# lightonai/next-plaid

Hardware: AMD Instinct MI355X
Metric: queries/sec + p50 latency, k=10, 10M-doc x 300-tok x d128 PLAID index, 1/2/4/8 GPU (higher is better)
Workload: dtype f32 (split-bf16 hi/lo MFMA on the residual term of MaxSim, f32-class accuracy)

## Files before the change

### next-plaid_amd/csrc/np_index.hip

```cpp
#include "np_internal.h"

#include <hipcub/hipcub.hpp>

#include <algorithm>
#include <memory>
#include <thread>
#include <math.h>
#include <stdio.h>
#include <time.h>
#include <stdlib.h>
#include <string.h>

namespace np {

int DevBuf::reserve(size_t bytes) {
  if (bytes <= cap) return NP_OK;
  if (p) (void)hipFree(p);
  p = nullptr;
  cap = 0;
  size_t want = bytes + (bytes >> 3) + 256;
  hipError_t e = hipMalloc(&p, want);
  if (e != hipSuccess) {
    p = nullptr;
    set_error("hipMalloc(%zu bytes) failed: %s", want, hipGetErrorString(e));
    return NP_ERR_OUT_OF_MEMORY;
  }
  cap = want;
  return NP_OK;
}
void DevBuf::release() {
  if (p) (void)hipFree(p);
  p = nullptr;
  cap = 0;
}

void shard_range(int64_t n_total, int rank, int count, int64_t* b, int64_t* e) {
  if (count <= 1) {
    *b = 0;
    *e = n_total;
    return;
  }
  *b = (int64_t)((__int128)n_total * rank / count);
  *e = (int64_t)((__int128)n_total * (rank + 1) / count);
}

int normalise_opts(const np_open_opts* in, np_open_opts* o) {
  memset(o, 0, sizeof *o);
  if (in) *o = *in;
  if (o->shard_count <= 0) o->shard_count = 1;
  if (o->shard_rank < 0 || o->shard_rank >= o->shard_count) {
    set_error("Invalid configuration: shard_rank %d out of range for shard_count %d", o->shard_rank, o->shard_count);
    return NP_ERR_INVALID_ARGUMENT;
  }
  if (o->n_contexts <= 0) o->n_contexts = 2;
  if (o->n_contexts > 16) o->n_contexts = 16;
  if (o->max_batch <= 0) o->max_batch = 64;
  if (o->max_query_tokens <= 0) o->max_query_tokens = 64;
  return NP_OK;
}

bool set_tuning(Tuning* t, const std::string& n, int value) {
  auto clamp = [](int v, int lo, int hi) { return std::min(std::max(v, lo), hi); };
  if (n == "s4_mode") t->s4_mode = clamp(value, 0, 8);
  else if (n == "s4_minb") t->s4_minb = std::max(value, 1);
  else if (n == "s4_nbx") t->s4_nbx = clamp(value, 8, 512);
  else if (n == "s4_swz") t->s4_swz = value != 0;
  else if (n == "s4_filter") t->s4_filter = value != 0;
  else if (n == "s4_hot") t->s4_hot = clamp(value, 0, 500);
  else if (n == "s4_planes") t->s4_planes = value != 0;
  else if (n == "s4_pexp") t->s4_pexp = clamp(value, 5, 40);
  else if (n == "s4_lpd") t->s4_lpd = value == 2 ? 2 : 4;
  else if (n == "s4_qm") t->s4_qm = value != 0;
  else if (n == "s4_pnbx") t->s4_pnbx = clamp(value, 8, 512);
  else if (n == "s3_slices") t->s3_slices = value != 0;
  else if (n == "s4_warm") t->s4_warm = clamp(value, 0, 1000);
  else if (n == "ub_ncut") t->ub_ncut = clamp(value, 1, 512);
  else if (n == "s3_bisect") t->s3_bisect = clamp(value, 0, 1);
  else if (n == "s3_gain") t->s3_gain = clamp(value, 0, 2);
  else if (n == "s3_gain_mult") t->s3_gain_mult = clamp(value, 1, 16);
  else if (n == "s3_gain_direct") t->s3_gain_direct = clamp(value, 0, 64);
  else if (n == "s4_hot_auto") t->s4_hot_auto = clamp(value, 0, 0x7fffffff);
  else if (n == "ub_nt") t->ub_nt = value < 0 || value > 2 ? 0 : value;
  else if (n == "ub_steal") t->ub_steal = value < 1 ? 1 : value;
  else if (n == "ub_nbx") t->ub_nbx = clamp(value, 8, 256);
  else if (n == "ub_direct") t->ub_direct = clamp(value, 0, 16);
#ifdef NP_DIAGNOSTICS
  else if (n == "s4_probe") t->s4_probe = clamp(value, 0, 7);
#endif
  else if (n == "ub_static") t->ub_static = value != 0;
  else if (n == "hot_static") t->hot_static = value != 0;
  else if (n == "s6_xcd") t->s6_xcd = value != 0;
  else if (n == "s6_tiles") t->s6_tiles = value != 0;
  else if (n == "s6_lds") t->s6_lds = clamp(value, 0, 2);
  else if (n == "gemm_cpw") t->gemm_cpw = value == 2 ? 2 : 1;
  else if (n == "s1_split") t->s1_split = value != 0;
  else if (n == "exact_rowmax") t->exact_rowmax = value != 0;
  else return false;
  return true;
}

void read_tuning_env(Tuning* t) {
  static const char* const knobs[][2] = {
      {"NP_S4_MODE", "s4_mode"}, {"NP_S4_MINB", "s4_minb"}, {"NP_S4_NBX", "s4_nbx"}, {"NP_S4_SWZ", "s4_swz"},
      {"NP_S4_FILTER", "s4_filter"}, {"NP_S4_HOT", "s4_hot"}, {"NP_S4_PLANES", "s4_planes"}, {"NP_S4_PEXP", "s4_pexp"}, {"NP_S4_LPD", "s4_lpd"}, {"NP_S4_QM", "s4_qm"}, {"NP_S4_PNBX", "s4_pnbx"}, {"NP_S4_WARM", "s4_warm"}, {"NP_UB_NCUT", "ub_ncut"}, {"NP_S3_BISECT", "s3_bisect"}, {"NP_S3_GAIN", "s3_gain"}, {"NP_S3_GAIN_MULT", "s3_gain_mult"}, {"NP_S3_GAIN_DIRECT", "s3_gain_direct"}, {"NP_S4_HOT_AUTO", "s4_hot_auto"}, {"NP_S3_SLICES", "s3_slices"}, {"NP_UB_NT", "ub_nt"},
      {"NP_UB_STEAL", "ub_steal"}, {"NP_UB_NBX", "ub_nbx"}, {"NP_UB_DIRECT", "ub_direct"}, {"NP_UB_STATIC", "ub_static"}, {"NP_HOT_STATIC", "hot_static"}, {"NP_S6_XCD", "s6_xcd"}, {"NP_S6_TILES", "s6_tiles"}, {"NP_S6_LDS", "s6_lds"}, {"NP_GEMM_CPW", "gemm_cpw"}, {"NP_S1_SPLIT", "s1_split"},
      {"NP_EXACT_ROWMAX", "exact_rowmax"}};
  for (const auto& k : knobs) {
    const char* e = getenv(k[0]);
    if (e && *e) (void)set_tuning(t, k[1], atoi(e));
  }
#ifdef NP_DIAGNOSTICS
  if (const char* e = getenv("NP_S4_PROBE")) (void)set_tuning(t, "s4_probe", atoi(e));
#endif
}

static void default_workspace(DeviceIndex* ix) {
  ix->ws_auto = ix->opts.workspace_bytes <= 0;
  ix->ws_budget = ix->opts.workspace_bytes;
  ix->ws_budget_open = ix->opts.workspace_bytes;
  if (!ix->ws_auto) return;
  size_t free_b = 0, total_b = 0;
  int64_t ws = (int64_t)8 << 30;
  if (hipMemGetInfo(&free_b, &total_b) == hipSuccess) {
    const int64_t share = ((int64_t)free_b - ((int64_t)4 << 30)) / std::max(ix->opts.n_contexts, 1);
    ws = std::min<int64_t>((int64_t)16 << 30, std::max<int64_t>((int64_t)2 << 30, share));
  }
  ix->opts.workspace_bytes = ws;
  ix->ws_budget = ws;
  ix->ws_budget_open = ws;
}

static int check_device(int dev) {
  int n = 0;
  if (hipGetDeviceCount(&n) != hipSuccess || n <= 0) {
    (void)hipGetLastError();
    set_error("no HIP device available");
    return NP_ERR_DEVICE_UNAVAILABLE;
  }
  if (dev < 0 || dev >= n) {
    set_error("device %d out of range (%d devices)", dev, n);
    return NP_ERR_DEVICE_UNAVAILABLE;
  }
  return NP_OK;
}

void destroy_device_index(np_index* ix) {
  if (!ix) return;
  DeviceGuard g(ix->device);
  for (Context* c : ix->contexts) destroy_context(c);
  delete ix;
}

struct CloseIndex {
  void operator()(np_index* p) const { destroy_device_index(p); }
};
using IndexHandle = std::unique_ptr<np_index, CloseIndex>;

static uint32_t bitrev(uint32_t v, int nbits) {
  uint32_t r = 0;
  for (int k = 0; k < nbits; ++k)
    if (v & (1u << k)) r |= 1u << (nbits - 1 - k);
  return r;
}

static int check_geometry(int64_t K, int dim, int nbits, int64_t n_total) {
  if (nbits <= 0 || 8 % nbits != 0) {
    set_error("Codec error: nbits must be a divisor of 8, got %d", nbits);
    return NP_ERR_CODEC;
  }
  if (K <= 0 || dim <= 0) {
    set_error("Shape error: centroids must be [K > 0, dim > 0], got [%lld, %d]", (long long)K, dim);
    return NP_ERR_SHAPE;
  }
  if ((dim * nbits) % 8 != 0) {
    set_error("Shape error: dim*nbits must be a multiple of 8 (dim=%d nbits=%d)", dim, nbits);
    return NP_ERR_SHAPE;
  }
  if (K >= ((int64_t)1 << 31) || n_total >= ((int64_t)1 << 32) - 1) {
    set_error("Index load failed: K=%lld / N=%lld exceed the 32-bit device id space", (long long)K, (long long)n_total);
    return NP_ERR_INDEX_LOAD;
  }
  return NP_OK;
}

__global__ void __launch_bounds__(256) centroid_bound_kernel(const float* __restrict__ C, int64_t K, int dim,
                                                             uint32_t* __restrict__ out ) {
  const int64_t c = (int64_t)blockIdx.x * 4 + (threadIdx.x >> 6);
// ... 1450 lines not shown
```

### next-plaid_amd/csrc/np_internal.h

```cpp
#pragma once
#include <hip/hip_runtime.h>
#include <stdint.h>
#include <algorithm>
#include <atomic>
#include <mutex>
#include <condition_variable>
#include <string>
#include <vector>
#include "../../include/nextplaid_hip.h"

namespace np {

struct CodeArr {
  const void* p;
  int wide;
  __device__ __forceinline__ uint32_t operator[](int64_t i) const {
    return wide ? static_cast<const uint32_t*>(p)[i] : (uint32_t)static_cast<const uint16_t*>(p)[i];
  }
};

void set_error(const char* fmt, ...) __attribute__((format(printf, 1, 2)));
const char* last_error();
void clear_error();

// ... 60 lines not shown
int build_check_finite(const float* x, int64_t count, int dim);
int find_outliers(int device, const float* X, int64_t n, int dim, const float* C, int64_t k, float thr,
                  std::vector<int64_t>* out, int64_t* n_rechecked);
int kmeans_points_as_docs(int device, const float* pts, int64_t n, int dim, const np_index_config& cfg, int64_t k,
                          std::vector<float>* cen);
int encode_with_codec(int device, const float* C, int64_t K, int dim, int nbits, const float* weights, const float* cutoffs,
                      const float* X, int64_t T, int64_t* codes, uint8_t* packed, float* norms);
float quantile_of_sorted(const std::vector<float>& v, double q);

template <class T>
class DevPtr {
 public:
  DevPtr() = default;
  DevPtr(DevPtr&& o) noexcept : p_(o.p_) { o.p_ = nullptr; }
  DevPtr& operator=(DevPtr&& o) noexcept {
    if (this != &o) {
      reset();
      p_ = o.p_;
      o.p_ = nullptr;
    }
    return *this;
  }
  ~DevPtr() { reset(); }
  int alloc(size_t n, size_t* acct = nullptr) {
    reset();
    const size_t bytes = std::max<size_t>(n, 1) * sizeof(T);
    hipError_t e = hipMalloc((void**)&p_, bytes);
    if (e != hipSuccess) {
      p_ = nullptr;
      set_error("hipMalloc(%zu bytes) failed: %s", bytes, hipGetErrorString(e));
      return NP_ERR_OUT_OF_MEMORY;
    }
    if (acct) *acct += bytes;
    return NP_OK;
  }
  T* get() const { return p_; }
  void reset() {
    if (p_) (void)hipFree(p_);
    p_ = nullptr;
  }

 private:
  T* p_ = nullptr;
};

struct DevBuf {
  void* p = nullptr;
  size_t cap = 0;
  int reserve(size_t bytes);
  void release();
  template <class T> T* as() const { return (T*)p; }
};

struct Workspace;

struct Context {
  hipStream_t stream = nullptr;
  hipEvent_t ev[10] = {};
  Workspace* ws = nullptr;
  bool busy = false;
  uint64_t last_use = 0;
};

struct Tuning {
  int s4_mode = 4;
  int s4_minb = 8;
  int s4_nbx = 128;
  int s4_swz = 1;
  int s3_bisect = 1;
  int s3_slices = 1;
  int s3_gain = 1;
  int s3_gain_mult = 3;
  int s3_gain_direct = 16;
  int s4_filter = 1;
  int s4_hot = 60;
  int s4_hot_auto = 200000;
  int s4_planes = 1;
  int s4_lpd = 2;
  int s4_pnbx = 96;
  int s4_qm = 1;
  int s4_pexp = 15;
  int s4_warm = 0;
  int ub_ncut = 96;
  int ub_direct = 8;
  int hot_static = 1;
  int ub_static = 0;
  int s4_probe = 0;
  int ub_nbx = 96;
  int ub_steal = 16384;
  int ub_nt = 2;
  int s6_xcd = 1;
  int s6_lds = 1;
  int s6_tiles = 1;
  int s1_split = 0;
  int gemm_cpw = 1;
  int exact_rowmax = 0;
};

#define NP_IVF_SPLIT_RANGE 32768

struct DeviceIndex {
  int device = 0;
  int64_t N_total = 0, n_emb_total = 0;
  double avg_doclen = 0.0;
  int64_t doc_begin = 0, n_docs = 0;
  int64_t K = 0, KP = 0;
  int32_t dim = 0, nbits = 0, pd = 0;
  int32_t ldim = 0, lnbits = 0, lpd = 0;
  float pad_ss = 0.f;
  int64_t T = 0;
  int64_t max_doc_len = 0;
  DevPtr<float> d_centroids;
  DevPtr<float> d_wlut;
  DevPtr<uint8_t> d_codes;
  int code_wide = 0;
  DevPtr<uint8_t> d_ucodes;
  int64_t n_ucodes = 0;
  int ublock_stride = 0;
  int ublock_hdr = 0;
  DevPtr<int32_t> d_ulen;
  DevPtr<uint4> d_useg;
  DevPtr<uint4> d_doc_meta;
  float ulen_mean = 0.f;
  bool sliced_ok = false;
  float cmax = 0.f;
  bool filter_ok = false;
  bool s6_fast_ok = false;
  DevPtr<float> d_inv_norm;
  DevPtr<uint16_t> d_tok_pos;
  bool tok_sorted = false;
  DevPtr<uint8_t> d_residuals;
  DevPtr<int64_t> d_doc_offsets;
  DevPtr<uint32_t> d_ivf;
  DevPtr<int64_t> d_ivf_offsets;
  int64_t ivf_size = 0;
  bool ivf_sorted = false;
  DevPtr<uint32_t> d_ivf_split;
  int n_ranges = 0;
  std::vector<int64_t> ivf_top_prefix;
  size_t device_bytes = 0;
  np_open_opts opts{};
  mutable std::atomic<int64_t> ws_budget{0};
  int64_t ws_budget_open = 0;
  bool ws_auto = false;
  Tuning tune;
  mutable std::atomic<int> gain_skip{0};
  mutable std::atomic<int> gain_run{0};
  mutable std::atomic<uint64_t> gain_key{0};
  CodeArr codes() const { return CodeArr{d_codes.get(), code_wide}; }
  CodeArr ucodes() const { return CodeArr{d_ucodes.get(), code_wide}; }
  size_t code_bytes() const { return code_wide ? 4 : 2; }
  mutable std::mutex mu;
  mutable std::condition_variable cv;
  mutable std::vector<Context*> contexts;
  mutable uint64_t use_clock = 0;
};

static inline int storage_dim(int dim) { return dim <= 0 || dim > 128 ? dim : (dim + 31) / 32 * 32; }
static inline int storage_nbits(int dim, int nbits) { return (nbits == 1 && dim <= 128) ? 2 : nbits; }

int build_device_index(const HostIndex& h, const np_open_opts* opts, DeviceIndex** out);
void destroy_device_index(np_index* ix);
int normalise_opts(const np_open_opts* in, np_open_opts* out);
void read_tuning_env(Tuning* t);
bool set_tuning(Tuning* t, const std::string& name, int value);
void shard_range(int64_t n_total, int rank, int count, int64_t* b, int64_t* e);
// ... 28 lines not shown
```

### next-plaid_amd/csrc/np_kernels.h

```cpp
#pragma once
#include <hip/hip_runtime.h>
#include <stdint.h>

namespace np {

typedef float f32x16 __attribute__((ext_vector_type(16)));
typedef __bf16 bf16x8 __attribute__((ext_vector_type(8)));

#define NP_NEG_INF (-__builtin_huge_valf())
#define NP_MAX_QT 8

__device__ __forceinline__ uint32_t okey(float x) {
  uint32_t b = __float_as_uint(x);
  uint32_t k = (b & 0x80000000u) ? ~b : (b | 0x80000000u);
  return ((b & 0x7F800000u) == 0x7F800000u) ? 0u : k;
}
__device__ __forceinline__ float unkey(uint32_t k) {
  uint32_t b = (k & 0x80000000u) ? (k ^ 0x80000000u) : ~k;
  return __uint_as_float(b);
}
__device__ __forceinline__ bool finitef(float x) { return (__float_as_uint(x) & 0x7F800000u) != 0x7F800000u; }
__device__ __forceinline__ float readlane_f(float v, int lane) {
  return __int_as_float(__builtin_amdgcn_readlane(__float_as_int(v), lane));
}
// ... 2418 lines not shown
          }
        };
        uint4 va[8], vb[8];
        issue(0, va);
        int t = 0;
        for (; t + 16 < np; t += 16) {
          issue(t + 8, vb);
          fold(va);
          issue(t + 16, va);
          fold(vb);
        }
        if (t + 8 < np) {
          issue(t + 8, vb);
          fold(va);
          fold(vb);
        } else {
          fold(va);
        }
      }
      uint32_t sum = 0;
      int slo = 0;
      if constexpr (FLOOR) {
        uint32_t fl = lam2;
        int lq_here = Lq - 16 * jl;
        asm volatile("" : "+v"(fl), "+v"(lq_here));
#pragma unroll
        for (int k = 0; k < 16; ++k) {
          slo += (int)st[k] - ((k < lq_here && st[k] <= 1u) ? 254 : 0);
          sum += max(st[k], k < lq_here ? fl : 0u);
        }
      } else {
#pragma unroll
        for (int k = 0; k < 16; ++k) {
          sum += st[k];
          slo += (int)st[k] - (st[k] == 1u ? 254 : 0);
        }
      }
#pragma unroll
      for (int o = 1; o < LPD; o <<= 1) {
        sum += (uint32_t)__shfl_xor((int)sum, o);
        slo += __shfl_xor(slo, o);
      }
      const uint32_t sum_lo = (uint32_t)max(slo, 0);
      if (valid && jl == 0) {
        U[pbase + i] = (uint16_t)sum;
        if (hb) atomicAdd(&s_hist[min(sum_lo >> hshift, (uint32_t)(NP_UB_BINS - 1))], 1u);
      }
      __builtin_amdgcn_wave_barrier();
    }
    __syncthreads();
    if (hb)
      for (int i = tid; i < NP_UB_BINS; i += 256) {
        const uint32_t v = s_hist[i];
        if (v) atomicAdd(&hb[i], v);
      }
  }
#pragma unroll
  for (int o = 32; o > 0; o >>= 1) {
    toks += __shfl_xor(toks, o);
    ucnt += __shfl_xor(ucnt, o);
    ndoc += __shfl_xor(ndoc, o);
  }
  __shared__ unsigned long long s_cnt[3];
  __syncthreads();
  if (tid == 0) s_cnt[0] = s_cnt[1] = s_cnt[2] = 0;
  __syncthreads();
  if (lane == 0 && toks) {
    atomicAdd(&s_cnt[0], toks);
    atomicAdd(&s_cnt[1], ucnt);
    atomicAdd(&s_cnt[2], ndoc);
  }
  __syncthreads();
  if (tid == 0 && s_cnt[0] && ctr) {
    if (count_tokens) {
      atomicAdd(&ctr->n_cand_tokens, s_cnt[0]);
      atomicAdd(&ctr->n_cand_dcodes, s_cnt[1]);
    } else {
      atomicAdd(&ctr->n_level2, s_cnt[2]);
    }
    atomicAdd(&ctr->n_cand_codes, s_cnt[1]);
  }
}

__global__ void __launch_bounds__(256) ub_thr_kernel(const uint32_t* __restrict__ hist, int hshift, int slack, int n_sel,
                                                     const int32_t* __restrict__ n_cand, RoundPlan rp, int round,
                                                     const uint32_t* __restrict__ qflag, uint32_t* __restrict__ thr) {
  __shared__ uint32_t s_part[256];
  constexpr int BPT = NP_UB_BINS / 256;
  const int b = blockIdx.x, tid = threadIdx.x;
  if (rp.round_of[b] != round) return;
  if (qflag[b] != 0 || n_cand[b] <= n_sel) {
    if (tid == 0) thr[b] = 0;
    return;
  }
  const uint32_t* hb = hist + (int64_t)b * NP_UB_BINS;
  const int top = (255 - tid) * BPT;
  uint32_t mine = 0;
#pragma unroll
  for (int k4 = 0; k4 < BPT / 4; ++k4) {
    const uint4 v = *reinterpret_cast<const uint4*>(hb + top + 4 * k4);
    mine += v.x + v.y + v.z + v.w;
  }
  s_part[tid] = mine;
  __syncthreads();
  if (tid == 0) {
    uint32_t cum = 0;
    int t = 0;
    for (; t < 255; ++t) {
      if (cum + s_part[t] >= (uint32_t)n_sel) break;
      cum += s_part[t];
    }
    int bin = (255 - t) * BPT + BPT - 1;
    for (; bin > (255 - t) * BPT; --bin) {
      if (cum + hb[bin] >= (uint32_t)n_sel) break;
      cum += hb[bin];
    }
    thr[b] = (uint32_t)max(0, bin - ((slack + (1 << hshift) - 1) >> hshift));
  }
}

struct CutP {
  const uint4* src;
  const int32_t* n_src_a;
  const int32_t* n_src_b;
  const uint16_t* U;
  const uint32_t* lo;
  const uint32_t* hi;
  int zero_mode;
  const uint4* all_src;
  const int32_t* n_all;
  uint4* dst;
  const int32_t* dst_begin;
  int32_t* n_dst;
  int hshift;
  Counters* ctr;
};

__global__ void __launch_bounds__(256) ub_cut_kernel(CutP p, RoundPlan rp, int round) {
  __shared__ int s_wcnt[4], s_base;
  __shared__ unsigned long long s_cnt[2];
  const int b = blockIdx.y, tid = threadIdx.x, lane = tid & 63, wave = tid >> 6;
  if (rp.round_of[b] != round) return;
  const uint32_t lo = p.lo[b], hi = p.hi ? p.hi[b] : 0xFFFFFFFFu;
  const bool all = lo == 0;
  if (all && p.zero_mode == 1) return;
  const uint4* src = all ? p.all_src : p.src;
  const int64_t n = all ? (int64_t)p.n_all[b] : (int64_t)p.n_src_a[b] + (p.n_src_b ? p.n_src_b[b] : 0);
  const int64_t pbase = rp.cand_base[b];
  const int64_t dbase = pbase + (p.dst_begin ? p.dst_begin[b] : 0);
  if (tid == 0) s_cnt[0] = s_cnt[1] = 0;
  unsigned long long toks = 0, ucnt = 0;
  constexpr int PT = 8;
  for (int64_t i0 = (int64_t)blockIdx.x * (256 * PT); i0 < n; i0 += (int64_t)gridDim.x * (256 * PT)) {
    bool keep[PT];
    unsigned long long bal[PT];
    int wtot = 0;
#pragma unroll
    for (int k = 0; k < PT; ++k) {
      const int64_t i = i0 + k * 256 + tid;
      bool kp = i < n;
      if (kp && !all) {
        const uint32_t bin = min((uint32_t)p.U[pbase + i] >> p.hshift, (uint32_t)(NP_UB_BINS - 1));
        kp = bin >= lo && bin < hi;
      }
      keep[k] = kp;
      bal[k] = __ballot(kp);
      wtot += (int)__popcll(bal[k]);
    }
    if (lane == 0) s_wcnt[wave] = wtot;
    __syncthreads();
    if (tid == 0) {
      const int tot = s_wcnt[0] + s_wcnt[1] + s_wcnt[2] + s_wcnt[3];
      s_base = tot ? atomicAdd(&p.n_dst[b], tot) : 0;
    }
    __syncthreads();
    int pos = s_base;
    for (int k = 0; k < wave; ++k) pos += s_wcnt[k];
#pragma unroll
    for (int k = 0; k < PT; ++k) {
      if (keep[k]) {
        const uint4 m = src[pbase + i0 + k * 256 + tid];
        p.dst[dbase + pos + (int)__popcll(bal[k] & ((1ull << lane) - 1ull))] = m;
        if (all) {
          toks += (unsigned long long)(m.w >> 8);
          ucnt += (unsigned long long)m.y;
        }
      }
      pos += (int)__popcll(bal[k]);
    }
    __syncthreads();
  }
  if (all && p.ctr) {
#pragma unroll
    for (int o = 32; o > 0; o >>= 1) {
      toks += __shfl_xor(toks, o);
      ucnt += __shfl_xor(ucnt, o);
    }
    if (lane == 0 && toks) {
      atomicAdd(&s_cnt[0], toks);
      atomicAdd(&s_cnt[1], ucnt);
    }
    __syncthreads();
    if (tid == 0 && s_cnt[0]) {
      atomicAdd(&p.ctr->n_cand_tokens, s_cnt[0]);
      atomicAdd(&p.ctr->n_cand_dcodes, s_cnt[1]);
      atomicAdd(&p.ctr->n_cand_codes, s_cnt[1]);
    }
  }
}

__global__ void __launch_bounds__(256) hot_prep_kernel(const uint8_t* __restrict__ QCU, int64_t K, int64_t KP, int RB,
                                                       uint8_t* __restrict__ cmaxu ,
                                                       uint32_t* __restrict__ chist ) {
  __shared__ uint32_t s_h[256];
  const int b = blockIdx.y, tid = threadIdx.x;
  s_h[tid] = 0;
  __syncthreads();
  for (int64_t c = (int64_t)blockIdx.x * 256 + tid; c < KP; c += (int64_t)gridDim.x * 256) {
    const uint4* row = reinterpret_cast<const uint4*>(QCU + ((int64_t)b * KP + c) * RB);
    uint32_t m = 0;
    for (int j = 0; j < RB / 16; ++j) {
      const uint4 v = row[j];
      const uint32_t w4[4] = {v.x, v.y, v.z, v.w};
#pragma unroll
      for (int e = 0; e < 4; ++e)
#pragma unroll
// ... 2455 lines not shown
```

### next-plaid_amd/csrc/np_search.hip

```cpp
#include "np_internal.h"
#include "np_kernels.h"

#include <algorithm>
#include <array>
#include <cmath>
#include <stdlib.h>
#include <string.h>
#include <type_traits>
#include <utility>

namespace np {

struct Workspace {
  DevBuf q, qoff, Qt, Qb, Qbl, QCT, gmax, tauq, cellbits, cells_tmp, cells, n_cells, docbits, chunk_counts, cand, cand_meta, approx, n_cand,
      cand_base, round_of, round_tab, QCU, qinv, qflag, ub, ub_hist, ub_thr, ub_cursor, q_order, xcd_slots, surv_meta, n_surv, n_list2, sel_keys, sel_doc, nsel, exact, out_ids, out_scores, out_keys, out_counts, ctr, subset,
      subset_bits, elig, misc, cut, cmaxu, chist, ub2, ub_hist2, ub_thr2, list_meta, n_l1, n_l2, qpad, planes, levels, hotbits,
      gain, gsmall, ghist, s0_meta, s0_u, gacc, gdeep;
  void* h_pin = nullptr;
  size_t h_pin_cap = 0;
  unsigned long long* h_gain = nullptr;
  uint64_t h_gain_key = 0;
  hipEvent_t done = nullptr;
  bool done_valid = false;
  static constexpr int NBUF = 66;
// ... 944 lines not shown
    hot_levels_kernel<<<dim3((unsigned)std::min<int64_t>(std::max<int64_t>((KP >> 5) / 256, 1), 16), B), 256, 0, st>>>(
        w.chist.as<uint32_t>(), ix->K, ix->tune.s4_hot, w.cmaxu.as<uint8_t>(), KP, ix->tune.s4_pexp, w.ub_thr2.as<uint32_t>() + B,
        w.levels.as<uint32_t>(), w.hotbits.as<uint32_t>(), p.s4_warm, w.ub_thr2.as<uint32_t>() + 2 * B,
        w.hotbits.as<uint32_t>() + (size_t)B * (KP / 32), ix->tune.s4_hot_auto ? w.n_cand.as<int32_t>() : nullptr,
        ix->tune.s4_hot_auto);
    const dim3 pg((unsigned)std::min<int64_t>((KP + 2047) / 2048, 64), B);
    with_int<32, 64>(p.RB, [&](auto RB) {
      hot_planes_kernel<RB><<<pg, 256, 0, st>>>(w.QCU.as<uint8_t>(), KP, w.cmaxu.as<uint8_t>(), w.ub_thr2.as<uint32_t>() + B,
                                                w.levels.as<uint32_t>(), w.planes.as<uint32_t>());
    });
  }
  return NP_OK;
}

int Pass::rounds(const RoundPlan& rp, const GainP& gp) const {
  SelectP sp;
  sp.approx = w.approx.as<float>();
  sp.cand = w.cand.as<uint32_t>();
  sp.cand_step = 1;
  sp.rp = rp;
  sp.n_cand = w.n_cand.as<int32_t>();
  sp.doc_begin = ix->doc_begin;
  sp.n_sel = cs->n_sel;
  sp.NSELP = cs->NSELP;
  sp.sel_keys = w.sel_keys.as<uint64_t>();
  sp.sel_doc = w.sel_doc.as<uint32_t>();
  sp.nsel_out = w.nsel.as<int32_t>();
  sp.ctr = nullptr;
  const size_t sel_lds = (size_t)cs->NSELP * 8;
  if (cs->n_sel > 0 && sel_lds > 48 * 1024)
    NP_HIP(hipFuncSetAttribute(reinterpret_cast<const void*>(&select_kernel),
                               hipFuncAttributeMaxDynamicSharedMemorySize, (int)sel_lds));
  for (int r = 0; r < (p.have_cands ? p.max_rounds : 0); ++r) NP_TRY(round(r, rp, gp, sp));
  return NP_OK;
}

int Pass::round(int r, const RoundPlan& rp, const GainP& gp, SelectP sp) const {
  const int B = p.B;
  if (p.gain_path)
    gain_emit_kernel<2><<<dim3((unsigned)ix->n_ranges, (unsigned)B), 256, 0, st>>>(gp, r);
  else
    compact_kernel<<<dim3(p.nchunks, B), 256, 0, st>>>(w.docbits.as<uint32_t>(), p.NW, p.nchunks, w.chunk_counts.as<int32_t>(),
                                                       (p.use_filter && !p.ids_only) ? nullptr : w.cand.as<uint32_t>(), rp, r,
                                                       p.ids_only ? nullptr : ix->d_doc_meta.get(), w.cand_meta.as<uint4>());
  if (cs->timed && r == 0) NP_HIP(hipEventRecord(cs->ctx->ev[3], st));
  const bool matvec = p.batched && !p.s1_split;
  if (p.use_filter) {
    NP_TRY(p.two_level ? two_level_cut(r, rp) : single_level_cut(r, rp));
    launch_approx(st, ix, w, d_qoff, B, p.LQP, w.surv_meta.as<uint4>(), w.n_surv.as<int32_t>(), rp, r, p.max_rounds, nullptr);
    sp.cand = reinterpret_cast<const uint32_t*>(w.surv_meta.p);
    sp.cand_step = 4;
    sp.n_cand = w.n_surv.as<int32_t>();
    sp.ctr = w.ctr.as<Counters>();
    if (matvec) {
      gcut_kernel<<<B, 1024, 0, st>>>(w.approx.as<float>(), w.surv_meta.as<uint4>(), w.n_surv.as<int32_t>(), rp, r, cs->n_sel,
                                      w.qinv.as<float>(), w.qflag.as<uint32_t>(), d_qoff, w.cand_meta.as<uint4>(),
                                      w.n_list2.as<int32_t>());
      launch_matvec(st, ix, w, d_q, d_qoff, B, w.cand_meta.as<uint4>(), w.n_list2.as<int32_t>(), rp, r);
      sp.cand = reinterpret_cast<const uint32_t*>(w.cand_meta.p);
      sp.n_cand = w.n_list2.as<int32_t>();
    }
  } else if (ix->T > 0) {
    if (matvec) {
      launch_matvec(st, ix, w, d_q, d_qoff, B, w.cand_meta.as<uint4>(), w.n_cand.as<int32_t>(), rp, r);
      count_work_kernel<<<dim3(32, (unsigned)B), 256, 0, st>>>(w.cand_meta.as<uint4>(), w.n_cand.as<int32_t>(), rp, r,
                                                               w.ctr.as<Counters>());
    } else {
      launch_approx(st, ix, w, d_qoff, B, p.LQP, w.cand_meta.as<uint4>(), w.n_cand.as<int32_t>(), rp, r, p.max_rounds,
                    w.ctr.as<Counters>());
    }
  }
  if (cs->timed && r == 0) NP_HIP(hipEventRecord(cs->ctx->ev[4], st));
  if (cs->n_sel > 0) {
    sp.round = r;
    select_kernel<<<B, 1024, (size_t)cs->NSELP * 8, st>>>(sp);
  }
  return NP_OK;
}

int Pass::single_level_cut(int r, const RoundPlan& rp) const {
  const int B = p.B;
  NP_TRY(ub_bounds(rp, r, p.max_rounds, slots((size_t)r * 3), cursor(0), w.cand_meta.as<uint4>(), nullptr, w.n_cand.as<int32_t>(),
                   w.n_cand.as<int32_t>(), w.ub.as<uint16_t>(), w.ub_hist.as<uint32_t>(), 1, 0, false));
  ub_thr_kernel<<<B, 256, 0, st>>>(w.ub_hist.as<uint32_t>(), p.hshift, p.slack, cs->n_sel, w.n_cand.as<int32_t>(), rp, r,
                                   w.qflag.as<uint32_t>(), w.ub_thr.as<uint32_t>());
  CutP cp{};
  cp.hshift = p.hshift;
  cp.all_src = w.cand_meta.as<uint4>();
  cp.n_all = w.n_cand.as<int32_t>();
  cp.src = w.cand_meta.as<uint4>();
  cp.n_src_a = w.n_cand.as<int32_t>();
  cp.U = w.ub.as<uint16_t>();
  cp.lo = w.ub_thr.as<uint32_t>();
  cp.zero_mode = 0;
  cp.dst = w.surv_meta.as<uint4>();
  cp.n_dst = w.n_surv.as<int32_t>();
  cp.ctr = w.ctr.as<Counters>();
  ub_cut_kernel<<<dim3(n_cut(), B), 256, 0, st>>>(cp, rp, r);
  return NP_OK;
}

int Pass::two_level_cut(int r, const RoundPlan& rp) const {
  const int B = p.B;
  const unsigned ncut = n_cut();
  auto ub = [&](int lvl, const int32_t* begin, const int32_t* count, int direct_wpq, bool floor_rows) {
    return ub_bounds(rp, r, p.max_rounds, slots((size_t)r * 3 + lvl), cursor(lvl), w.list_meta.as<uint4>(), begin, count,
                     w.n_cand.as<int32_t>(), w.ub2.as<uint16_t>(), w.ub_hist2.as<uint32_t>(), 0, direct_wpq, floor_rows);
  };
  CutP cp{};
  cp.hshift = p.hshift;
  cp.all_src = w.cand_meta.as<uint4>();
  cp.n_all = w.n_cand.as<int32_t>();
  if (cs->timed && r == 0) NP_HIP(hipEventRecord(cs->ctx->ev[8], st));
  NP_TRY(hot_level(r, rp));
  if (cs->timed && r == 0) {
    NP_HIP(hipEventRecord(cs->ctx->ev[9], st));
    cs->hot_timed = true;
  }
  ub_thr_kernel<<<B, 256, 0, st>>>(w.ub_hist.as<uint32_t>(), p.hshift, 0, cs->n_sel, w.n_cand.as<int32_t>(), rp, r,
                                   w.qflag.as<uint32_t>(), w.ub_thr.as<uint32_t>());
  cp.src = w.cand_meta.as<uint4>();
  cp.n_src_a = w.n_cand.as<int32_t>();
  cp.U = w.ub.as<uint16_t>();
  cp.lo = w.ub_thr.as<uint32_t>();
  cp.zero_mode = 1;
  cp.dst = w.list_meta.as<uint4>();
  cp.n_dst = w.n_l1.as<int32_t>();
  ub_cut_kernel<<<dim3(ncut, B), 256, 0, st>>>(cp, rp, r);
  NP_TRY(ub(1, nullptr, w.n_l1.as<int32_t>(), ix->tune.ub_direct, false));
  ub_thr_kernel<<<B, 256, 0, st>>>(w.ub_hist2.as<uint32_t>(), p.hshift, p.slack, cs->n_sel, w.n_cand.as<int32_t>(), rp, r,
                                   w.qflag.as<uint32_t>(), w.ub_thr2.as<uint32_t>());
  cp.lo = w.ub_thr2.as<uint32_t>();
  cp.hi = w.ub_thr.as<uint32_t>();
  cp.dst_begin = w.n_l1.as<int32_t>();
  cp.n_dst = w.n_l2.as<int32_t>();
  ub_cut_kernel<<<dim3(ncut, B), 256, 0, st>>>(cp, rp, r);
  NP_TRY(ub(2, w.n_l1.as<int32_t>(), w.n_l2.as<int32_t>(), 0, true));
  ub_thr_kernel<<<B, 256, 0, st>>>(w.ub_hist2.as<uint32_t>(), p.hshift, p.slack, cs->n_sel, w.n_cand.as<int32_t>(), rp, r,
                                   w.qflag.as<uint32_t>(), w.ub_thr2.as<uint32_t>());
  cp.src = w.list_meta.as<uint4>();
  cp.n_src_a = w.n_l1.as<int32_t>();
  cp.n_src_b = w.n_l2.as<int32_t>();
  cp.U = w.ub2.as<uint16_t>();
  cp.lo = w.ub_thr2.as<uint32_t>();
  cp.hi = nullptr;
  cp.zero_mode = 0;
  cp.dst = w.surv_meta.as<uint4>();
  cp.dst_begin = nullptr;
  cp.n_dst = w.n_surv.as<int32_t>();
  cp.ctr = w.ctr.as<Counters>();
  ub_cut_kernel<<<dim3(ncut, B), 256, 0, st>>>(cp, rp, r);
  return NP_OK;
}

int Pass::hot_level(int r, const RoundPlan& rp) const {
  const int B = p.B;
  const int64_t KP = p.KP;
  const int old_cap = ix->code_wide ? 64 : 128;
  const int plpd = (ix->ublock_stride > old_cap || ix->tune.s4_lpd == 4) ? 4 : 2;
  const unsigned pnbx = (unsigned)ix->tune.s4_pnbx;
  return with_codes(ix->code_wide, [&](auto ct) -> int {
    using CT = decltype(ct);
    if (!p.use_planes) {
      return with_rowb(p.RB, [&](auto RB) -> int {
        int32_t* sl = slots((size_t)r * 3);
        const size_t dyn = (size_t)(KP / 8);
        if (dyn > 16 * 1024)
          NP_HIP(hipFuncSetAttribute(reinterpret_cast<const void*>(&approx_hot_kernel<RB, CT>),
                                     hipFuncAttributeMaxDynamicSharedMemorySize, (int)dyn));
        approx_hot_kernel<RB, CT><<<8 * (unsigned)ix->tune.ub_nbx, 256, dyn, st>>>(
            w.QCU.as<uint8_t>(), ix->K, KP, w.cmaxu.as<uint8_t>(), w.ub_thr2.as<uint32_t>() + B, w.cand.as<uint32_t>(),
            w.cand_meta.as<uint4>(), ix->ublock_stride, (int64_t)ix->n_docs * ix->ublock_stride, w.n_cand.as<int32_t>(), rp, r,
            p.max_rounds, (const CT*)ix->d_ucodes.get(), w.qflag.as<uint32_t>(), d_qoff, cs->n_sel, w.ub.as<uint16_t>(),
            w.ub_hist.as<uint32_t>(), p.hshift, cursor(0), sl, sl + 8 * (B + 1), B, ix->tune.ub_steal, w.ctr.as<Counters>(),
            ix->tune.s4_probe, ix->tune.hot_static);
        return NP_OK;
      });
    }
    return with_int<32, 64>(p.RB, [&](auto RB) -> int {
      const int sb = ix->ublock_stride * (int)sizeof(CT);
      if constexpr (sizeof(CT) == 4) {
        if ((KP >> 3) >= 32 * 1024 && plpd == 4 && sb > 240 && sb <= 496)
          return hotp<RB, CT, 4, 1, 2, 0, 12>(r, rp, 32);
      }
      if (plpd == 2) {
        if (sb <= 240 && ix->tune.s4_qm) return hotp<RB, CT, 2, 2, 4, 1>(r, rp, pnbx);
        if (sb <= 240) return hotp<RB, CT, 2, 2, 4, 0>(r, rp, pnbx);
        return hotp<RB, CT, 2, 2, 2, 0>(r, rp, pnbx);
      }
      if (sb <= 240) return hotp<RB, CT, 4, 1, 4, 0>(r, rp, pnbx);
      if (sb <= 496) return hotp<RB, CT, 4, 1, 2, 0>(r, rp, pnbx);
      return hotp<RB, CT, 4, 1, 1, 0>(r, rp, pnbx);
    });
  });
}

template <int RB, class CT, int LPD, int PF, int DPI, int QM, int WPB>
int Pass::hotp(int r, const RoundPlan& rp, unsigned nbx) const {
  const int B = p.B;
  const int64_t KP = p.KP;
  int32_t* sl = slots((size_t)r * 3);
  const size_t bm = sizeof(CT) == 2 ? 0 : (size_t)(((KP >> 5) + 3) & ~(int64_t)3) * 4;
  const size_t rowb = (size_t)ix->ublock_stride * sizeof(CT) + 16;
  const int slack = (int)std::max<int64_t>(256, 1024 - (int64_t)DPI * (int64_t)rowb);
  const size_t dynp = bm + (size_t)WPB * ((64 / LPD) * rowb + (size_t)slack);
  if (dynp > 16 * 1024)
    NP_HIP(hipFuncSetAttribute(reinterpret_cast<const void*>(&approx_hotp_kernel<RB, CT, LPD, PF, DPI, QM, WPB>),
                               hipFuncAttributeMaxDynamicSharedMemorySize, (int)dynp));
  approx_hotp_kernel<RB, CT, LPD, PF, DPI, QM, WPB><<<8 * nbx, 64 * WPB, dynp, st>>>(
      w.planes.as<uint32_t>(), ix->K, KP, w.hotbits.as<uint32_t>(), w.ub_thr2.as<uint32_t>() + B, w.levels.as<uint32_t>(),
      w.cand.as<uint32_t>(), w.cand_meta.as<uint4>(), ix->ublock_stride, (int64_t)ix->n_docs * ix->ublock_stride,
      w.n_cand.as<int32_t>(), rp, r, p.max_rounds, (const CT*)ix->d_ucodes.get(), w.qflag.as<uint32_t>(), d_qoff, cs->n_sel,
      w.ub.as<uint16_t>(), w.ub_hist.as<uint32_t>(), p.hshift, sl, sl + 8 * (B + 1), B, w.ctr.as<Counters>(), slack,
      ix->tune.s4_probe, p.gain_path ? 1 : 0);
  return NP_OK;
}

static int phase_a_once(const DeviceIndex* ix, CallState* cs, const float* d_q, const int32_t* d_qoff,
                        const int32_t* h_qoff, const int64_t* d_subset, int64_t subset_len, bool allow_grow) {
  Workspace& w = *cs->ctx->ws;
  hipStream_t st = cs->stream;
  PassPlan p;
  NP_TRY(plan_pass(ix, cs, h_qoff, subset_len, allow_grow, p));
  NP_TRY(reserve_pass(ix, cs, p, w));
  settle_zeroth_level(ix, w, cs, p);
  if (ix->ldim != ix->dim) {
    if (p.rows > 0)
// ... 791 lines not shown
```

Measured before the change: 20610.

## Fuse UB threshold computation into cut kernel and parallelize threshold scan

Removes the separate ub_thr_kernel launches by computing each query's histogram threshold inside ub_cut_kernel, with block 0 writing it back for later stages. The threshold search becomes a wave-level shuffle prefix scan instead of a serial single-thread loop. It also adds an s4_s1_mult knob for first-level sampling and sizes the direct workgroups-per-query from the sample count, raising the ub_direct clamp to 64. The cost is that every cut block redundantly reads the histogram and repeats the scan.

```diff
diff --git a/next-plaid_amd/csrc/np_index.hip b/next-plaid_amd/csrc/np_index.hip
--- a/next-plaid_amd/csrc/np_index.hip
+++ b/next-plaid_amd/csrc/np_index.hip
@@ -74,6 +74,7 @@
   else if (n == "s4_pnbx") t->s4_pnbx = clamp(value, 8, 512);
   else if (n == "s3_slices") t->s3_slices = value != 0;
   else if (n == "s4_warm") t->s4_warm = clamp(value, 0, 1000);
+  else if (n == "s4_s1_mult") t->s4_s1_mult = clamp(value, 1, 8);
   else if (n == "ub_ncut") t->ub_ncut = clamp(value, 1, 512);
   else if (n == "s3_bisect") t->s3_bisect = clamp(value, 0, 1);
   else if (n == "s3_gain") t->s3_gain = clamp(value, 0, 2);
@@ -83,7 +84,7 @@
   else if (n == "ub_nt") t->ub_nt = value < 0 || value > 2 ? 0 : value;
   else if (n == "ub_steal") t->ub_steal = value < 1 ? 1 : value;
   else if (n == "ub_nbx") t->ub_nbx = clamp(value, 8, 256);
-  else if (n == "ub_direct") t->ub_direct = clamp(value, 0, 16);
+  else if (n == "ub_direct") t->ub_direct = clamp(value, 0, 64);
 #ifdef NP_DIAGNOSTICS
   else if (n == "s4_probe") t->s4_probe = clamp(value, 0, 7);
 #endif
@@ -102,7 +103,7 @@
 void read_tuning_env(Tuning* t) {
   static const char* const knobs[][2] = {
       {"NP_S4_MODE", "s4_mode"}, {"NP_S4_MINB", "s4_minb"}, {"NP_S4_NBX", "s4_nbx"}, {"NP_S4_SWZ", "s4_swz"},
-      {"NP_S4_FILTER", "s4_filter"}, {"NP_S4_HOT", "s4_hot"}, {"NP_S4_PLANES", "s4_planes"}, {"NP_S4_PEXP", "s4_pexp"}, {"NP_S4_LPD", "s4_lpd"}, {"NP_S4_QM", "s4_qm"}, {"NP_S4_PNBX", "s4_pnbx"}, {"NP_S4_WARM", "s4_warm"}, {"NP_UB_NCUT", "ub_ncut"}, {"NP_S3_BISECT", "s3_bisect"}, {"NP_S3_GAIN", "s3_gain"}, {"NP_S3_GAIN_MULT", "s3_gain_mult"}, {"NP_S3_GAIN_DIRECT", "s3_gain_direct"}, {"NP_S4_HOT_AUTO", "s4_hot_auto"}, {"NP_S3_SLICES", "s3_slices"}, {"NP_UB_NT", "ub_nt"},
+      {"NP_S4_FILTER", "s4_filter"}, {"NP_S4_HOT", "s4_hot"}, {"NP_S4_PLANES", "s4_planes"}, {"NP_S4_PEXP", "s4_pexp"}, {"NP_S4_LPD", "s4_lpd"}, {"NP_S4_QM", "s4_qm"}, {"NP_S4_PNBX", "s4_pnbx"}, {"NP_S4_WARM", "s4_warm"}, {"NP_S4_S1_MULT", "s4_s1_mult"}, {"NP_UB_NCUT", "ub_ncut"}, {"NP_S3_BISECT", "s3_bisect"}, {"NP_S3_GAIN", "s3_gain"}, {"NP_S3_GAIN_MULT", "s3_gain_mult"}, {"NP_S3_GAIN_DIRECT", "s3_gain_direct"}, {"NP_S4_HOT_AUTO", "s4_hot_auto"}, {"NP_S3_SLICES", "s3_slices"}, {"NP_UB_NT", "ub_nt"},
       {"NP_UB_STEAL", "ub_steal"}, {"NP_UB_NBX", "ub_nbx"}, {"NP_UB_DIRECT", "ub_direct"}, {"NP_UB_STATIC", "ub_static"}, {"NP_HOT_STATIC", "hot_static"}, {"NP_S6_XCD", "s6_xcd"}, {"NP_S6_TILES", "s6_tiles"}, {"NP_S6_LDS", "s6_lds"}, {"NP_GEMM_CPW", "gemm_cpw"}, {"NP_S1_SPLIT", "s1_split"},
       {"NP_EXACT_ROWMAX", "exact_rowmax"}};
   for (const auto& k : knobs) {
diff --git a/next-plaid_amd/csrc/np_internal.h b/next-plaid_amd/csrc/np_internal.h
--- a/next-plaid_amd/csrc/np_internal.h
+++ b/next-plaid_amd/csrc/np_internal.h
@@ -166,6 +166,7 @@
   int s4_pexp = 15;
   int s4_warm = 0;
   int ub_ncut = 96;
+  int s4_s1_mult = 1;
   int ub_direct = 8;
   int hot_static = 1;
   int ub_static = 0;
diff --git a/next-plaid_amd/csrc/np_kernels.h b/next-plaid_amd/csrc/np_kernels.h
--- a/next-plaid_amd/csrc/np_kernels.h
+++ b/next-plaid_amd/csrc/np_kernels.h
@@ -2524,41 +2524,66 @@
   }
 }
 
+__device__ __forceinline__ uint32_t ub_thr_block(const uint32_t* __restrict__ hb, int hshift, int slack, uint32_t n_reach,
+                                                 uint32_t* s_w) {
+  constexpr int BPT = NP_UB_BINS / 256;
+  const int tid = threadIdx.x, lane = tid & 63, wave = tid >> 6;
+  const int top = (255 - tid) * BPT;
+  uint32_t h[BPT];
+#pragma unroll
+  for (int k4 = 0; k4 < BPT / 4; ++k4) {
+    const uint4 v = *reinterpret_cast<const uint4*>(hb + top + 4 * k4);
+    h[4 * k4] = v.x; h[4 * k4 + 1] = v.y; h[4 * k4 + 2] = v.z; h[4 * k4 + 3] = v.w;
+  }
+  uint32_t mine = 0;
+#pragma unroll
+  for (int k = 0; k < BPT; ++k) mine += h[k];
+  uint32_t inc = mine;
+#pragma unroll
+  for (int o = 1; o < 64; o <<= 1) {
+    const uint32_t v = (uint32_t)__shfl_up((int)inc, o);
+    if (lane >= o) inc += v;
+  }
+  if (lane == 63) s_w[wave] = inc;
+  if (tid == 0) s_w[4] = 0;
+  __syncthreads();
+  for (int k = 0; k < wave; ++k) inc += s_w[k];
+  uint32_t cum = inc - mine;
+  if (cum < n_reach && inc >= n_reach) {
+    int bin = top;
+    bool found = false;
+#pragma unroll
+    for (int k = BPT - 1; k >= 1; --k) {
+      if (!found) {
+        if (cum + h[k] >= n_reach) {
+          bin = top + k;
+          found = true;
+        } else {
+          cum += h[k];
+        }
+      }
+    }
+    s_w[4] = (uint32_t)max(0, bin - ((slack + (1 << hshift) - 1) >> hshift));
+  }
+  __syncthreads();
+  return s_w[4];
+}
+
+__device__ __forceinline__ uint32_t ub_thr_query(const uint32_t* __restrict__ hist, int b, int hshift, int slack, int n_reach,
+                                                 int n_sel, const int32_t* __restrict__ n_cand,
+                                                 const uint32_t* __restrict__ qflag, uint32_t* s_w) {
+  if (qflag[b] != 0 || n_cand[b] <= n_sel) return 0u;
+  return ub_thr_block(hist + (int64_t)b * NP_UB_BINS, hshift, slack, (uint32_t)n_reach, s_w);
+}
+
 __global__ void __launch_bounds__(256) ub_thr_kernel(const uint32_t* __restrict__ hist, int hshift, int slack, int n_sel,
                                                      const int32_t* __restrict__ n_cand, RoundPlan rp, int round,
                                                      const uint32_t* __restrict__ qflag, uint32_t* __restrict__ thr) {
-  __shared__ uint32_t s_part[256];
-  constexpr int BPT = NP_UB_BINS / 256;
-  const int b = blockIdx.x, tid = threadIdx.x;
+  __shared__ uint32_t s_w[5];
+  const int b = blockIdx.x;
   if (rp.round_of[b] != round) return;
-  if (qflag[b] != 0 || n_cand[b] <= n_sel) {
-    if (tid == 0) thr[b] = 0;
-    return;
-  }
-  const uint32_t* hb = hist + (int64_t)b * NP_UB_BINS;
-  const int top = (255 - tid) * BPT;
-  uint32_t mine = 0;
-#pragma unroll
-  for (int k4 = 0; k4 < BPT / 4; ++k4) {
-    const uint4 v = *reinterpret_cast<const uint4*>(hb + top + 4 * k4);
-    mine += v.x + v.y + v.z + v.w;
-  }
-  s_part[tid] = mine;
-  __syncthreads();
-  if (tid == 0) {
-    uint32_t cum = 0;
-    int t = 0;
-    for (; t < 255; ++t) {
-      if (cum + s_part[t] >= (uint32_t)n_sel) break;
-      cum += s_part[t];
-    }
-    int bin = (255 - t) * BPT + BPT - 1;
-    for (; bin > (255 - t) * BPT; --bin) {
-      if (cum + hb[bin] >= (uint32_t)n_sel) break;
-      cum += hb[bin];
-    }
-    thr[b] = (uint32_t)max(0, bin - ((slack + (1 << hshift) - 1) >> hshift));
-  }
+  const uint32_t t = ub_thr_query(hist, b, hshift, slack, n_sel, n_sel, n_cand, qflag, s_w);
+  if (threadIdx.x == 0) thr[b] = t;
 }
 
 struct CutP {
@@ -2566,7 +2591,11 @@
   const int32_t* n_src_a;
   const int32_t* n_src_b;
   const uint16_t* U;
-  const uint32_t* lo;
+  const uint32_t* hist;
+  int slack, n_reach;
+  int n_sel;
+  const uint32_t* qflag;
+  uint32_t* lo;
   const uint32_t* hi;
   int zero_mode;
   const uint4* all_src;
@@ -2581,9 +2610,12 @@
 __global__ void __launch_bounds__(256) ub_cut_kernel(CutP p, RoundPlan rp, int round) {
   __shared__ int s_wcnt[4], s_base;
   __shared__ unsigned long long s_cnt[2];
+  __shared__ uint32_t s_thr[5];
   const int b = blockIdx.y, tid = threadIdx.x, lane = tid & 63, wave = tid >> 6;
   if (rp.round_of[b] != round) return;
-  const uint32_t lo = p.lo[b], hi = p.hi ? p.hi[b] : 0xFFFFFFFFu;
+  const uint32_t lo = ub_thr_query(p.hist, b, p.hshift, p.slack, p.n_reach, p.n_sel, p.n_all, p.qflag, s_thr);
+  const uint32_t hi = p.hi ? p.hi[b] : 0xFFFFFFFFu;
+  if (blockIdx.x == 0 && tid == 0) p.lo[b] = lo;
   const bool all = lo == 0;
   if (all && p.zero_mode == 1) return;
   const uint4* src = all ? p.all_src : p.src;
diff --git a/next-plaid_amd/csrc/np_search.hip b/next-plaid_amd/csrc/np_search.hip
--- a/next-plaid_amd/csrc/np_search.hip
+++ b/next-plaid_amd/csrc/np_search.hip
@@ -1050,8 +1050,6 @@
   const int B = p.B;
   NP_TRY(ub_bounds(rp, r, p.max_rounds, slots((size_t)r * 3), cursor(0), w.cand_meta.as<uint4>(), nullptr, w.n_cand.as<int32_t>(),
                    w.n_cand.as<int32_t>(), w.ub.as<uint16_t>(), w.ub_hist.as<uint32_t>(), 1, 0, false));
-  ub_thr_kernel<<<B, 256, 0, st>>>(w.ub_hist.as<uint32_t>(), p.hshift, p.slack, cs->n_sel, w.n_cand.as<int32_t>(), rp, r,
-                                   w.qflag.as<uint32_t>(), w.ub_thr.as<uint32_t>());
   CutP cp{};
   cp.hshift = p.hshift;
   cp.all_src = w.cand_meta.as<uint4>();
@@ -1059,6 +1057,10 @@
   cp.src = w.cand_meta.as<uint4>();
   cp.n_src_a = w.n_cand.as<int32_t>();
   cp.U = w.ub.as<uint16_t>();
+  cp.hist = w.ub_hist.as<uint32_t>();
+  cp.slack = p.slack;
+  cp.n_reach = cp.n_sel = cs->n_sel;
+  cp.qflag = w.qflag.as<uint32_t>();
   cp.lo = w.ub_thr.as<uint32_t>();
   cp.zero_mode = 0;
   cp.dst = w.surv_meta.as<uint4>();
@@ -1079,38 +1081,42 @@
   cp.hshift = p.hshift;
   cp.all_src = w.cand_meta.as<uint4>();
   cp.n_all = w.n_cand.as<int32_t>();
+  cp.n_sel = cs->n_sel;
+  cp.qflag = w.qflag.as<uint32_t>();
   if (cs->timed && r == 0) NP_HIP(hipEventRecord(cs->ctx->ev[8], st));
   NP_TRY(hot_level(r, rp));
   if (cs->timed && r == 0) {
     NP_HIP(hipEventRecord(cs->ctx->ev[9], st));
     cs->hot_timed = true;
   }
-  ub_thr_kernel<<<B, 256, 0, st>>>(w.ub_hist.as<uint32_t>(), p.hshift, 0, cs->n_sel, w.n_cand.as<int32_t>(), rp, r,
-                                   w.qflag.as<uint32_t>(), w.ub_thr.as<uint32_t>());
+  const int n_sample = ix->tune.s4_s1_mult * cs->n_sel;
   cp.src = w.cand_meta.as<uint4>();
   cp.n_src_a = w.n_cand.as<int32_t>();
   cp.U = w.ub.as<uint16_t>();
+  cp.hist = w.ub_hist.as<uint32_t>();
+  cp.slack = 0;
+  cp.n_reach = n_sample;
   cp.lo = w.ub_thr.as<uint32_t>();
   cp.zero_mode = 1;
   cp.dst = w.list_meta.as<uint4>();
   cp.n_dst = w.n_l1.as<int32_t>();
   ub_cut_kernel<<<dim3(ncut, B), 256, 0, st>>>(cp, rp, r);
-  NP_TRY(ub(1, nullptr, w.n_l1.as<int32_t>(), ix->tune.ub_direct, false));
-  ub_thr_kernel<<<B, 256, 0, st>>>(w.ub_hist2.as<uint32_t>(), p.hshift, p.slack, cs->n_sel, w.n_cand.as<int32_t>(), rp, r,
-                                   w.qflag.as<uint32_t>(), w.ub_thr2.as<uint32_t>());
+  const int per_wg = 4 * 64 / (p.RB / 16);
+  const int wpq = ix->tune.ub_direct > 0 ? std::min(64, std::max(ix->tune.ub_direct, (n_sample + per_wg - 1) / per_wg)) : 0;
+  NP_TRY(ub(1, nullptr, w.n_l1.as<int32_t>(), wpq, false));
+  cp.hist = w.ub_hist2.as<uint32_t>();
+  cp.slack = p.slack;
+  cp.n_reach = cs->n_sel;
   cp.lo = w.ub_thr2.as<uint32_t>();
   cp.hi = w.ub_thr.as<uint32_t>();
   cp.dst_begin = w.n_l1.as<int32_t>();
   cp.n_dst = w.n_l2.as<int32_t>();
   ub_cut_kernel<<<dim3(ncut, B), 256, 0, st>>>(cp, rp, r);
   NP_TRY(ub(2, w.n_l1.as<int32_t>(), w.n_l2.as<int32_t>(), 0, true));
-  ub_thr_kernel<<<B, 256, 0, st>>>(w.ub_hist2.as<uint32_t>(), p.hshift, p.slack, cs->n_sel, w.n_cand.as<int32_t>(), rp, r,
-                                   w.qflag.as<uint32_t>(), w.ub_thr2.as<uint32_t>());
   cp.src = w.list_meta.as<uint4>();
   cp.n_src_a = w.n_l1.as<int32_t>();
   cp.n_src_b = w.n_l2.as<int32_t>();
   cp.U = w.ub2.as<uint16_t>();
-  cp.lo = w.ub_thr2.as<uint32_t>();
   cp.hi = nullptr;
   cp.zero_mode = 0;
   cp.dst = w.surv_meta.as<uint4>();
```

New measurement: 20250. -1.7%, worse.
